# ZJU-FAST-Lab/uneven_planner

Hardware: AMD Instinct MI355X
Metric: MINCO traj-opts/sec (batch) (higher is better)
Workload: dtype f64

## Files before the change

uneven_planner_amd/csrc/solver_program.hpp:

```cpp
#pragma once
#include "terrain_dev.hpp"
#include "trajectory_dev.hpp"
#include "uph_common.hpp"

namespace uph {

#ifndef UPH_GRID_FROM_MEM
#define UPH_GRID_FROM_MEM 1
#endif
#ifndef UPH_PHASE_MASK
#define UPH_PHASE_MASK 15
#endif
#ifndef UPH_STATE_PROBE
#define UPH_STATE_PROBE(st) do { } while (0)
#endif
#ifndef UPH_SCALING_WB
#define UPH_SCALING_WB 8
#endif
#ifndef UPH_SC_XB
#define UPH_SC_XB 9
#endif
#ifndef UPH_SC_YB
#define UPH_SC_YB 14
#endif
#ifndef UPH_SC_WLO
#define UPH_SC_WLO 2
#endif
#ifndef UPH_SC_WHI
#define UPH_SC_WHI 3
#endif

#ifndef UPH_ASIDE_PREP
#define UPH_ASIDE_PREP 1
#endif
template <class WG, class F>
UPH_HD void asideKnotSolve(WG& wg, int lenW, int lenX, int n, F f) {
    (void)lenW; (void)lenX;
    wg.pfor(n, f);
}

template <class WG, class SR = double>
struct Solver {
    WG& wg;
    const GridDev& grid;
    const OptParams& P;
    const BatchDev& bd;
    const TrajDesc& td;
    int Nxy, Nyaw, n, S, K, mem, CH, CHP, recd;
    int CHS;
    int* rtag;
    double *x, *xp, *g, *gp, *d, *cxy, *cyaw, *Gxy, *Gyaw, *gamxy, *gamyaw, *bt, *rec, *wtab, *ttab, *pf, *hd;
    double* ab;
    int* abn;
    static constexpr int AB_DOUBLES = 4;
    double* up;
    static constexpr int UP_DOUBLES = 6;
    UPH_HD void tally(int k, bool yes) {
#if defined(__HIP_DEVICE_COMPILE__)
        if (yes && wg.wave == 0) abn[k] = abn[k] + 1;
#else
        if (yes) abn[k]++;
#endif
    }
    double *dual, *res, *scl, *hist;
    int hrow, hnp;
    const double *Wr_xy, *Wr_yaw;
    double rho, scale_fx, Txy, Tyaw, last_jerk, last_gd;
    long long hist_reads;
    long long cyc[16];
    long long t_last_eval_end;
    long long* sub_t = nullptr;
    int evals, bidx, trace_n;
    float inv_k1;
    double ec_irho, ec_step, ec_invK, ec_iTyaw, ec_omega, ec_omega_h;

    static constexpr int REC_FIELDS = 12;
    static UPH_HD size_t ldsDoubles(int Nxy, int Nyaw, int n, int CH, int mem, int K) {
        size_t recd = (size_t)REC_FIELDS * (CH + 1) + (CH + 1) / 2;
        const size_t nvec = 2 * (Nxy + 5) + (Nyaw + 5);
        const size_t knd = (size_t)knotBufDoubles(Nxy + 1, 4) + knotBufDoubles(Nyaw + 1, 2), adj = (size_t)knotBufDoubles(Nxy, 4) + knotBufDoubles(Nyaw, 2) + nvec;
        recd = recd < knd ? knd : recd;
        recd = recd < adj ? adj : recd;
        recd = recd < (size_t)mem ? (size_t)mem : recd;
        const size_t td_ = (size_t)Nxy + K + 2;
        return (size_t)5 * n + (nvec < td_ ? td_ : nvec) + 2 * (12 * Nxy + 6 * Nyaw) + recd + (size_t)6 * (K + 1) + THOMAS_DOUBLES + MAX_PAST + 8 + 18 + AB_DOUBLES + UP_DOUBLES;
    }

    UPH_HD Solver(WG& w, const GridDev& gr, const OptParams& p, const BatchDev& b, int bi, double* lds)
        : wg(w), grid(gr), P(p), bd(b), td(b.desc[bi]) {
        bidx = bi;
        Nxy = td.Nxy; Nyaw = td.Nyaw; n = td.n; S = td.S; K = P.int_K; mem = P.mem_size;
        inv_k1 = 1.0f / (float)(K + 1);
        CH = wg.size(); CHP = CH + 1; recd = REC_FIELDS * CHP + (CH + 1) / 2;
        CHS = CH;
#if !defined(UPH_ALIGNED_CHUNKS) || UPH_ALIGNED_CHUNKS
        {
            const int ppc = CH / (K + 1);
            if (ppc >= 1 && (Nxy + ppc - 1) / ppc == (S + CH - 1) / CH) CHS = ppc * (K + 1);
        }
#endif
        double* q = lds;
        x = q; q += n; g = q; q += n; d = q; q += n;
        xp = q; q += n; gp = q; q += n;
        const int nvec = 2 * (Nxy + 5) + (Nyaw + 5);
        bt = q;
        gamxy = q; gamyaw = q + 2 * (Nxy + 5);
        q += nvec < Nxy + K + 2 ? Nxy + K + 2 : nvec;
        cxy = q; q += 12 * Nxy; cyaw = q; q += 6 * Nyaw;
        Gxy = q; q += 12 * Nxy; Gyaw = q; q += 6 * Nyaw;
        wtab = q; q += 6 * (K + 1);
        rec = q;
        {
            size_t rd = (size_t)recd;
            const size_t knd = (size_t)knotBufDoubles(Nxy + 1, 4) + knotBufDoubles(Nyaw + 1, 2), adj = (size_t)knotBufDoubles(Nxy, 4) + knotBufDoubles(Nyaw, 2) + nvec;
            rd = rd < knd ? knd : rd; rd = rd < adj ? adj : rd; rd = rd < (size_t)mem ? (size_t)mem : rd;
            q += rd;
        }
        rtag = (int*)(rec + (size_t)REC_FIELDS * CHP);
        ttab = q; q += THOMAS_DOUBLES;
        pf = q; q += MAX_PAST + 8;
        hd = q; q += 18;
        ab = q; q += AB_DOUBLES;
        abn = (int*)(ab + 1);
        up = q; q += UP_DOUBLES;
        dual = bd.dual + 7 * td.off_s; res = bd.res + 7 * td.off_s; scl = bd.scl + 7 * td.off_s;
        hist = bd.hist + td.off_hist; hrow = histRowDoubles(n); hnp = 64 * histNQ(n);
        Wr_xy = bd.ops[td.op_xy].Wr; Wr_yaw = bd.ops[td.op_yaw].Wr;
        rho = 0; scale_fx = 1.0; Txy = Tyaw = 0; last_jerk = 0; hist_reads = 0; evals = 0; trace_n = 0;
        for (int q = 0; q < 16; q++) cyc[q] = 0;
        t_last_eval_end = 0;
        wg.pfor(18 + THOMAS_DOUBLES, [&](int t) {
            if (t == 0) { ab[0] = 0.0; abn[0] = abn[1] = abn[2] = abn[3] = 0; }
            if (t < 18) hd[t] = t < 6 ? td.init_xy[t] : (t < 12 ? td.end_xy[t - 6] : (t < 15 ? td.init_yaw[t - 12] : td.end_yaw[t - 15]));
            else ttab[t - 18] = bd.thomas[t - 18];
        });
    }

    UPH_HD void tracePush(double v) {
        if (bd.trace != nullptr && trace_n < bd.trace_cap) {
            const int at = trace_n;
            wg.one([&]() { bd.trace[(size_t)bidx * bd.trace_cap + at] = v; });
        }
        trace_n++;
    }

    static UPH_HD int divSmall(int a, int b, float inv) {
        int q = (int)((float)a * inv);
        const int r = a - q * b;
        if (r < 0) q--;
        else if (r >= b) q++;
        return q;
    }
    static UPH_HD int knotCol(int j, int N) { return j == 0 ? 0 : (j == N ? N + 2 : j + 2); }
    UPH_HD double knotPos(const double* xin, int j, int dd) const {
        if (dd < 2) return j == 0 ? hd[dd] : (j == Nxy ? hd[6 + dd] : xin[1 + 2 * (j - 1) + dd]);
        return j == 0 ? hd[12] : (j == Nyaw ? hd[15] : xin[1 + 2 * (Nxy - 1) + (j - 1)]);
    }

    UPH_HD double dot(const double* a, const double* b, int m) {
// ... 996 lines not shown
            step = io->step; fx = io->fx; k = io->k; end = io->end; bound = io->bound; budget = io->budget;
            wg.pfor(n, [&](int i) { xp[i] = x[i]; gp[i] = g[i]; });
            dginit = dot(g, d, n);
        } else {
            fx = eval<false>(x, g);
            wg.pfor(n + 1, [&](int i) { if (i < n) { d[i] = -g[i]; xp[i] = x[i]; gp[i] = g[i]; } else pf[0] = fx; });
            const double gnorm0 = absmax(g, n), xnorm0 = absmax(x, n);
            if (gnorm0 / dmax(1.0, xnorm0) < P.g_epsilon) {
                ret = LBFGS_CONVERGENCE;
                run = false;
            } else {
                const double dd0 = dot(d, d, n);
                step = 1.0 / sqrt(dd0);
                dginit = -dd0;
                k = 1; end = 0; bound = 0;
            }
        }
        double gnorm_inf, xnorm_inf;
        if (run) {
            while (true) {
                if constexpr (RESUME) {
                    if (budget == 0) { ret = LBFGS_RUNNING_HOOK; break; }
                    budget--;
                }
                ls = lineSearch(fx, step, P.min_step, P.max_step, dginit);
                if (ls < 0) {
                    wg.pfor(n, [&](int i) { x[i] = xp[i]; g[i] = gp[i]; });
                    ret = ls;
                    break;
                }
                tracePush(fx);
                if (k > 1000) { ret = LBFGS_CANCELED; break; }
                double* hr = hist + (size_t)end * hrow;
                double* sc = hr + 2;
                double* yc = hr + 2 + hnp;
                const double pf_old = (0 < P.past && P.past <= k) ? wg.bcast(pf[k % P.past]) : 0.0;
                UPH_MARK("lbfgs.bookkeeping");
                double r5[5], mx2[2];
                wg.template sumMax<5, 2>(n, r5, mx2, [&](int i, double* acc, double* mx) {
                    const double xv = x[i], gv = g[i], xo = xp[i], go = gp[i];
                    const double sv = xv - xo, yv = gv - go;
                    mx[0] = dmax(mx[0], fabs(gv)); mx[1] = dmax(mx[1], fabs(xv));
                    sc[i] = sv; yc[i] = yv;
                    acc[0] += yv * sv; acc[1] += yv * yv; acc[2] += sv * sv; acc[3] += go * go; acc[4] += gv * gv;
                    xp[i] = xv; gp[i] = gv;
                    d[i] = -gv;
                });
                gnorm_inf = mx2[0];
                xnorm_inf = mx2[1];
                if (gnorm_inf / dmax(1.0, xnorm_inf) < P.g_epsilon) { ret = LBFGS_CONVERGENCE; break; }
                if (0 < P.past) {
                    if (P.past <= k) {
                        const double rate = fabs(pf_old - fx) / dmax(1.0, fabs(fx));
                        if (rate < P.delta) { ret = LBFGS_STOP; break; }
                    }
                }
                if (P.inner_max_iter != 0 && P.inner_max_iter <= k) { ret = LBFGSERR_MAXIMUMITERATION; break; }
                ys = r5[0]; yy = r5[1];
                const double cau = r5[2] * sqrt(r5[3]) * P.cautious_factor;
                {
                    const int kk = k, e0 = end;
                    const double fv = fx, ysv = ys;
                    wg.pfor(1, [&](int) {
                        if (0 < P.past) pf[kk % P.past] = fv;
                        double* h0 = hist + (size_t)e0 * hrow;
                        h0[0] = ysv; h0[1] = 1.0 / ysv;
                    });
                }
// ... 151 lines not shown
            st.f = io.fx; st.last_lbfgs_ret = ret; st.lbfgs_iters = io.k;
        });
        storeTrajectory(st);
    }

    UPH_HD void microbench(TrajState& st, int reps) {
        const double* gx0 = bd.x + td.off_x;
        rho = wg.bcast(st.rho); scale_fx = wg.bcast(st.scale_fx);
        wg.pfor(n, [&](int t) { x[t] = gx0[t]; d[t] = 0.5; xp[t] = gx0[t]; gp[t] = 0.25; });
        long long a[9];
        long long sub[8] = {0, 0, 0, 0, 0, 0, 0, 0};
        sub_t = sub;
        double acc = 0.0, js[3], part[3], c1, c2;
        const int cnt = S < CH ? S : CH;
        a[0] = wg.clock();
        for (int r = 0; r < reps; r++) generate<false>(x, 0.0);
        a[1] = wg.clock();
        for (int r = 0; r < reps; r++) { expand(x, 1.0, js); acc += js[0]; }
        a[2] = wg.clock();
        for (int r = 0; r < reps; r++) evalConsts(evalStep());
        a[3] = wg.clock();
        for (int r = 0; r < reps; r++) { wg.template sum<3>(cnt, part, [&](int t, double* ac) { sampleEval<false>(t, t, ac); }); acc += part[0]; }
        a[4] = wg.clock();
        for (int r = 0; r < reps; r++) scatterChunk(0, cnt);
        a[5] = wg.clock();
        for (int r = 0; r < reps; r++) { adjoint(c1, c2); acc += c1 + c2; }
        a[6] = wg.clock();
        const int m = mem;
        for (int r = 0; r < reps; r++) {
            const int end = (r * 7) % m, bound = m;
            acc += absmax(g, n) + absmax(x, n);
            wg.sync();
            wg.pfor(1, [&](int) { pf[r % 3] = acc; });
            double* sc = hist + (size_t)end * hrow + 2;
            double* yc = sc + hnp;
            double r6[6] = {0, 0, 0, 0, 0, 0};
            wg.template sum<3>(n, r6, [&](int i, double* ac) {
                const double sv = x[i] - xp[i], yv = g[i] - gp[i];
                sc[i] = sv; yc[i] = yv;
                ac[0] += yv * sv; ac[1] += yv * yv; ac[2] += sv * sv;
                d[i] = -g[i];
            });
            acc += r6[0] + r6[3] + sqrt(dot(gp, gp, n));
            wg.sync();
            wg.pfor(1, [&](int) { hist[(size_t)end * hrow] = acc; });
            (void)bound;
        }
        a[7] = wg.clock();
        wg.pfor(1, [&](int) {
            for (int q = 0; q < 7; q++) st.cyc[q] = (a[q + 1] - a[q]) / reps;
            st.cyc[7] = a[7] - a[0];
            for (int q = 0; q < 8; q++) st.cyc[8 + q] = sub[q] / reps;
            st.f = acc;
        });
        sub_t = nullptr;
    }

    UPH_HD void evalOnly(TrajState& st, int repeat) {
        const double* gx0 = bd.x + td.off_x;
        rho = wg.bcast(st.rho); scale_fx = wg.bcast(st.scale_fx);
        wg.pfor(n, [&](int t) { x[t] = gx0[t]; });
        double f = 0.0;
        for (int r = 0; r < repeat; r++) f = eval<false>(x, g);
        refreshResiduals();
        wg.pfor(n, [&](int t) { bd.gout[td.off_x + t] = g[t]; });
        storeTrajectory(st);
        wg.pfor(1, [&](int) { st.f = f; });
    }
// ... 89 lines not shown
```

uneven_planner_amd/csrc/unevenhip.hip:

```cpp
#include <hip/hip_runtime.h>

#include <type_traits>

#include <algorithm>
#include <cmath>
#include <cstdio>
#include <cstdlib>
#include <cstring>
#include <map>
#include <numeric>
#include <string>
#include <thread>
#include <vector>

#include "../../include/uneven_hip.h"
#include "minco_op_host.hpp"
#include "resample_walk.hpp"
#include "solver_program.hpp"
#include "uph_ctx.hpp"
#include "wave_dev.hpp"

using namespace uph;

#ifndef UPH_THOMAS_KPL
// ... 181 lines not shown
#pragma unroll
            for (int w = 1; w < NW; w++) t += r[w * MAXM + m];
            outS[m] = uni(t);
        }
#pragma unroll
        for (int m = 0; m < MM; m++) {
            double t = r[MS + m];
#pragma unroll
            for (int w = 1; w < NW; w++) t = r[w * MAXM + MS + m] > t ? r[w * MAXM + MS + m] : t;
            outM[m] = uni(t);
        }
    }
    __device__ __forceinline__ double bcast(double v) const { return uni(v); }
    static __device__ __forceinline__ double divByStored(double x, double ys, double r) {
        const double q0 = x * r;
        return fma(fma(-q0, ys, x), r, q0);
    }
    template <int NQ, int PF>
    __device__ __forceinline__ void twoLoopT(double* d, const double* g, double* dg_out, double* al_lds, int n_, const double* hist_, int m_, int end_, int bound_, double scale_) {
        typedef double dbl2_t __attribute__((ext_vector_type(2)));
        typedef const __attribute__((address_space(1))) char* gbytes;
        constexpr int NP2 = NQ / 2;
        constexpr bool ODD = (NQ & 1) != 0;
        constexpr int NPAD = 64 * NQ, ROWB = (2 + 2 * NPAD) * 8;
        const gbytes hist = (gbytes)uniG(hist_);
        const int lane = flane();
        const int n = uni(n_), m = uni(m_), end = uni(end_), bound = uni(bound_);
        const double scale = uni(scale_);
        const unsigned l16 = 16u * (unsigned)lane, l8 = 8u * (unsigned)lane;
        auto eidx = [&](int q) { return q < 2 * NP2 ? 128 * (q >> 1) + 2 * lane + (q & 1) : 64 * (NQ - 1) + lane; };
        double dr[NQ], sr[PF][NQ], yr[PF][NQ], ysr[PF], rysr[PF];
#pragma unroll
        for (int q = 0; q < NQ; q++) { const int e = eidx(q); dr[q] = e < n ? d[e] : 0.0; }
        auto fetch = [&](int slot, int j) {
            const gbytes row = hist + (size_t)((unsigned)j * (unsigned)ROWB);
            const dbl2_t yr2 = *(const __attribute__((address_space(1))) dbl2_t*)row;
            ysr[slot] = yr2.x; rysr[slot] = yr2.y;
#pragma unroll
            for (int p = 0; p < NP2; p++) {
                const dbl2_t s2 = *(const __attribute__((address_space(1))) dbl2_t*)(row + 16 + 1024 * p + l16);
                const dbl2_t y2 = *(const __attribute__((address_space(1))) dbl2_t*)(row + 16 + NPAD * 8 + 1024 * p + l16);
                sr[slot][2 * p] = s2.x; sr[slot][2 * p + 1] = s2.y; yr[slot][2 * p] = y2.x; yr[slot][2 * p + 1] = y2.y;
            }
            if (ODD) {
                sr[slot][NQ - 1] = *(const __attribute__((address_space(1))) double*)(row + 16 + 512 * (NQ - 1) + l8);
                yr[slot][NQ - 1] = *(const __attribute__((address_space(1))) double*)(row + 16 + NPAD * 8 + 512 * (NQ - 1) + l8);
            }
        };
        auto rowDot = [&](const double* a, const double* b_) {
            if (NQ == 1) return a[0] * b_[0];
            if (NQ == 2) return fma(a[1], b_[1], a[0] * b_[0]);
            if (NQ == 3) return fma(a[2], b_[2], fma(a[1], b_[1], a[0] * b_[0]));
            if (NQ == 4) return fma(a[1], b_[1], a[0] * b_[0]) + fma(a[3 % NQ], b_[3 % NQ], a[2 % NQ] * b_[2 % NQ]);
            double e = a[0] * b_[0], o = a[1 % NQ] * b_[1 % NQ];
#pragma unroll
            for (int q = 2; q < NQ; q += 2) e = fma(a[q], b_[q], e);
#pragma unroll
            for (int q = 3; q < NQ; q += 2) o = fma(a[q], b_[q], o);
            return e + o;
        };
        auto step1 = [&](int u, int i) {
            const double al = divByStored(waveSum(rowDot(sr[u], dr)), ysr[u], rysr[u]);
            al_lds[i] = al;
#pragma unroll
            for (int q = 0; q < NQ; q++) dr[q] = fma(-al, yr[u][q], dr[q]);
        };
        auto step2 = [&](int u, int i) {
            const double alpha = al_lds[bound - 1 - i];
            const double beta = divByStored(waveSum(rowDot(yr[u], dr)), ysr[u], rysr[u]);
            const double a = alpha - beta;
#pragma unroll
            for (int q = 0; q < NQ; q++) dr[q] = fma(a, sr[u][q], dr[q]);
        };
        auto pin = [&]() {
#pragma unroll
            for (int q = 0; q < NQ; q++) asm volatile("" : "+v"(dr[q]) : : "memory");
        };
#ifdef UPH_TL_PROF
        const long long tp0 = __builtin_readcyclecounter();
#endif
        int jf = end;
// ... 181 lines not shown
            __builtin_amdgcn_s_setprio(3);
            constexpr int PF = UPH_TWOLOOP_PF;
            const int nq = uni((n + 63) >> 6);
            if (nq == 1) twoLoopT<1, PF>(d, g, dg_out, al_lds, n, hist, m, end, bound, scale);
            else if (nq == 2) twoLoopT<2, PF>(d, g, dg_out, al_lds, n, hist, m, end, bound, scale);
            else if (nq == 3) twoLoopT<3, PF>(d, g, dg_out, al_lds, n, hist, m, end, bound, scale);
            else if (nq == 4) twoLoopT<4, PF>(d, g, dg_out, al_lds, n, hist, m, end, bound, scale);
            else if (nq == 5) twoLoopT<5, 2>(d, g, dg_out, al_lds, n, hist, m, end, bound, scale);
            else if (nq == 6) twoLoopT<6, 2>(d, g, dg_out, al_lds, n, hist, m, end, bound, scale);
            else if (nq == 7) twoLoopT<7, 2>(d, g, dg_out, al_lds, n, hist, m, end, bound, scale);
            else twoLoopT<8, 2>(d, g, dg_out, al_lds, n, hist, m, end, bound, scale);
            __builtin_amdgcn_s_setprio(0);
        }
        bar(1);
    }
    template <class F>
    __device__ __forceinline__ double maxv(int n, F f) {
        double a = 0.0;
        for (int i = ftid(); i < n; i += NT) { const double v = f(i); a = v > a ? v : a; }
        a = waveMax(a);
        double* r = red + par * (NW * MAXM);
        par ^= 1;
        if (lane == 0) r[wave * MAXM] = a;
        bar(0);
        double t = r[0];
#pragma unroll
        for (int w = 1; w < NW; w++) t = r[w * MAXM] > t ? r[w * MAXM] : t;
        return uni(t);
    }
};

template <int NT, class F>
__device__ __forceinline__ void asideKnotSolve(DevWG<NT>& wg, int lenW, int lenX, int n, F f) { wg.aside(lenW, lenX, n, f); }

template <int NT, int WPS, int MODE, bool F32S = false>
__global__ __launch_bounds__(NT, WPS) void uph_solver_kernel(GridDev grid, OptParams P, BatchDev bd, int repeat) {
    extern __shared__ double lds[];
    const int w = blockIdx.x;
    if (w >= bd.B) return;
    const int b = bd.order ? bd.order[w] : w;
    DevWG<NT> wg(lds);
    typedef typename std::conditional<F32S, f32r, double>::type SR;
    Solver<DevWG<NT>, SR> sol(wg, grid, P, bd, b, lds + DevWG<NT>::SCRATCH);
    TrajState& st = bd.state[b];
    if (MODE == 0) sol.evalOnly(st, repeat);
    else if (MODE == 1) sol.prepare(st);
    else if (MODE == 2) sol.optimize(st, repeat);
    else if (MODE == 7) sol.resumeHook(st, repeat >> 1, repeat & 1);
    else if (MODE == 8) { if (repeat & 1) sol.template penaltyOnly<true>(st, repeat >> 1); else sol.template penaltyOnly<false>(st, repeat >> 1); }
    else if (MODE == 3) sol.report(st);
    else if (MODE == 5) sol.microbench(st, repeat);
    else sol.scalingOnly(st);
}

__global__ void uph_fill_kernel(double* __restrict__ p, size_t n, double v) {
    for (size_t i = (size_t)blockIdx.x * blockDim.x + threadIdx.x; i < n; i += (size_t)gridDim.x * blockDim.x) p[i] = v;
}

__global__ void uph_terrain_kernel(GridDev grid, const double* __restrict__ pos, int n, double* __restrict__ values, double* __restrict__ grads) {
    const int i = blockIdx.x * blockDim.x + threadIdx.x;
    if (i >= n) return;
    const double yaw = pos[3 * i + 2];
    double v[7], g[7][3];
    terrainAllWithGrad(grid, pos[3 * i], pos[3 * i + 1], yaw, cos(yaw), sin(yaw), v, g);
    for (int k = 0; k < 7; k++) {
        values[7 * i + k] = v[k];
// ... 253 lines not shown
        else if (mode == 2) UPH_LAUNCH(NTL, WPS, 2);                                                                                 \
        else if (mode == 3) UPH_LAUNCH(NTL, WPS, 3);                                                                                 \
        else if (mode == 5) UPH_LAUNCH(NTL, WPS, 5);                                                                                 \
        else UPH_LAUNCH(NTL, WPS, 4);                                                                                                \
    } while (0)
#define UPH_LAUNCH32(NTL, WPS, MODE)                                                                                                   \
    do {                                                                                                                             \
        const size_t ldsmax = 160 * 1024;    \
        HIPCHK(hipFuncSetAttribute((const void*)uph_solver_kernel<NTL, WPS, MODE, true>, hipFuncAttributeMaxDynamicSharedMemorySize, (int)ldsmax)); \
        HIPCHK(hipEventRecord(evb, c->stream));                                                                                   \
        BatchDev bm = bd;                                                                                                            \
        bm.B = c->n_main;                                                                                                            \
        if (c->n_main < c->B) {                                                                                                      \
            BatchDev bb = bd;                                                                                                        \
            bb.B = c->B - c->n_main;                                                                                                 \
            bb.order = bd.order + c->n_main;                                                                                         \
            HIPCHK(hipStreamWaitEvent(c->stream2, evb, 0));                                                                       \
            hipLaunchKernelGGL((uph_solver_kernel<NTL, WPS, MODE, true>), dim3(bb.B), dim3(NTL), c->lds_big, c->stream2, grid, c->P, bb, repeat); \
            HIPCHK(hipEventRecord(c->ev2, c->stream2));                                                                              \
        }                                                                                                                            \
        hipLaunchKernelGGL((uph_solver_kernel<NTL, WPS, MODE, true>), dim3(c->n_main), dim3(NTL), c->lds_bytes, c->stream, grid, c->P, bm, repeat); \
        if (c->n_main < c->B) HIPCHK(hipStreamWaitEvent(c->stream, c->ev2, 0));                                                      \
    } while (0)
    if (c->sample_f32 && (mode == 0 || mode == 2) && (c->lanes == 128 || c->lanes == 256 || c->lanes == 512)) {
        if (c->lanes == 128) { if (mode == 0) UPH_LAUNCH32(128, 2, 0); else UPH_LAUNCH32(128, 2, 2); }
        else if (c->lanes == 512) { if (mode == 0) UPH_LAUNCH32(512, 1, 0); else UPH_LAUNCH32(512, 1, 2); }
        else if (mode == 0) UPH_LAUNCH32(256, 1, 0);
        else if (c->wps == 2 && c->lds_bytes <= 80 * 1024) UPH_LAUNCH32(256, 2, 2);
        else UPH_LAUNCH32(256, 1, 2);
    }
    else if (mode == 7) {
        if (c->lanes == 128) UPH_LAUNCH(128, 2, 7);
        else if (c->lanes == 256) UPH_LAUNCH(256, 1, 7);
        else { setError("the L-BFGS resume hook is built for 128 and 256 lanes"); return UPH_ERR_INVALID; }
    }
    else if (mode == 8) {
        if (c->lanes == 128) UPH_LAUNCH(128, 2, 8);
        else if (c->lanes == 256) UPH_LAUNCH(256, 1, 8);
        else if (c->lanes == 512) UPH_LAUNCH(512, 1, 8);
        else UPH_LAUNCH(64, 1, 8);
    }
    else if (c->lanes == 64 && c->wps_forced == 2) UPH_LAUNCH_MODE(64, 2);
    else if (c->lanes == 64) UPH_LAUNCH_MODE(64, 1);
    else if (c->lanes == 128 && mode == 1) UPH_LAUNCH(128, 1, 1);
    else if (c->lanes == 128) UPH_LAUNCH_MODE(128, UPH_WPS128);
    else if (c->lanes == 512) UPH_LAUNCH_MODE(512, 1);
    else if (c->wps == 2 && mode == 2 && c->lds_bytes <= 80 * 1024) UPH_LAUNCH(256, 2, 2);
    else if (c->wps == 2 && mode == 5 && c->lds_bytes <= 80 * 1024) UPH_LAUNCH(256, 2, 5);
    else UPH_LAUNCH_MODE(256, 1);
#undef UPH_LAUNCH_MODE
#undef UPH_LAUNCH32
#undef UPH_LAUNCH
    HIPCHK(hipGetLastError());
    if (mode == 0 || mode == 2 || mode == 4 || mode == 7) c->traj_resident = true;
    HIPCHK(hipEventRecord(eve, c->stream));
    if (async) return UPH_OK;
    HIPCHK(hipStreamSynchronize(c->stream));
    float ms = 0.f;
    HIPCHK(hipEventElapsedTime(&ms, evb, eve));
    c->last_ms = ms;
    return UPH_OK;
}

static int uploadPackedX(uph_ctx* c, const double* x_packed) {
    if (c->frames.empty()) { HIPCHK(hipMemcpy(c->d_x.p, x_packed, 8 * c->sum_n, hipMemcpyHostToDevice)); return UPH_OK; }
    std::vector<double> xl(x_packed, x_packed + c->sum_n);
    for (int b = 0; b < c->B; b++) {
// ... 188 lines not shown
    c->frames.clear();
    c->framed_valid = false;
    c->frames_grid = tg;
    if (std::max(std::max(std::fabs(tg.minb[0]), std::fabs(tg.maxb[0])), std::max(std::fabs(tg.minb[1]), std::fabs(tg.maxb[1]))) > FRAME_EXTENT) {
        c->frames.resize(B);
        for (int b = 0; b < B; b++) {
            const ProblemHead& q = *pp[b];
            TrajFrame& f = c->frames[b];
            const int nn[2] = {tg.nx, tg.ny};
            for (int d = 0; d < 2; d++) {
                long long ci = std::llround((0.5 * (q.lo[d] + q.hi[d]) - tg.origin[d]) * tg.xy_inv);
                ci = ci < 0 ? 0 : (ci > nn[d] ? nn[d] : ci);
                f.ioff[d] = (int)ci;
                f.shift[d] = tg.origin[d] + (double)ci * tg.xy_res;
                f.fo[d] = 0.0;
                f.lo[d] = tg.lo[d] - f.shift[d];
                f.hi[d] = tg.hi[d] - f.shift[d];
            }
        }
    }
    for (int b = 0; b < B; b++) {
        const ProblemHead& pr = *pp[b];
        const int Nxy = pr.n_inner_xy + 1, Nyaw = pr.n_inner_yaw + 1;
        TrajDesc& t = c->desc[b];
        std::memset(&t, 0, sizeof(t));
        t.Nxy = Nxy; t.Nyaw = Nyaw; t.n = 2 * pr.n_inner_xy + pr.n_inner_yaw + 1; t.S = Nxy * K1;
        t.op_xy = ensureOp(c, Nxy);
        t.op_yaw = ensureOp(c, Nyaw);
        if (t.op_xy < 0 || t.op_yaw < 0) return UPH_ERR_HIP;
        t.off_x = on; t.off_s = os; t.off_cxy = ocx; t.off_cyaw = ocy; t.off_hist = oh;
        for (int k = 0; k < 6; k++) { t.init_xy[k] = pr.init_xy[k]; t.end_xy[k] = pr.end_xy[k]; }
        for (int k = 0; k < 3; k++) { t.init_yaw[k] = pr.init_yaw[k]; t.end_yaw[k] = pr.end_yaw[k]; }
        if (!c->frames.empty()) for (int d = 0; d < 2; d++) { t.init_xy[d] -= c->frames[b].shift[d]; t.end_xy[d] -= c->frames[b].shift[d]; }
        on += t.n; os += t.S; ocx += 12 * Nxy; ocy += 6 * Nyaw; oh += (int64_t)mem * histRowDoubles(t.n);
        c->fp_bytes[b] = (Solver<DevWG<64>>::ldsDoubles(Nxy, Nyaw, t.n, c->lanes, mem, c->P.int_K) + 2 * (c->lanes / 64) * DevWG<64>::MAXM) * sizeof(double);
        lds_d = std::max(lds_d, Solver<DevWG<64>>::ldsDoubles(Nxy, Nyaw, t.n, c->lanes, mem, c->P.int_K));
    }
    c->sum_n = on; c->sum_S = os; c->sum_cxy = ocx; c->sum_cyaw = ocy; c->sum_hist = oh;
    c->lds_bytes = (lds_d + 2 * (c->lanes / 64) * DevWG<64>::MAXM) * sizeof(double);
    if (c->lds_bytes > 160 * 1024) { setError("uph_batch_upload: trajectory does not fit the 160 KiB LDS"); return UPH_ERR_LIMIT; }
    if (c->ops_dirty) {
        if (c->d_ops.ensure(sizeof(MincoOp) * c->ops_host.size())) return UPH_ERR_HIP;
        HIPCHK(hipMemcpy(c->d_ops.p, c->ops_host.data(), sizeof(MincoOp) * c->ops_host.size(), hipMemcpyHostToDevice));
        c->ops_dirty = false;
    }
    if (c->d_desc.ensure(sizeof(TrajDesc) * B) || c->d_state.ensure(sizeof(TrajState) * B) || c->d_x.ensure(8 * on) || c->d_x0.ensure(8 * on) || c->d_gout.ensure(8 * on) ||
        c->d_dual.ensure(8 * 7 * os) || c->d_res.ensure(8 * 7 * os) || c->d_scl.ensure(8 * 7 * os) || c->d_cxy.ensure(8 * ocx) || c->d_cyaw.ensure(8 * ocy) ||
        c->d_hist.ensure(8 * oh) || c->d_report.ensure(8 * 7 * B) || c->d_order.ensure(4 * B) ||
        c->d_trace.ensure(8 * (size_t)std::max(1, c->trace_cap) * B))
        return UPH_ERR_HIP;
    {
        std::vector<double> cost(B);
        for (int b = 0; b < B; b++) cost[b] = predictedCostOf(pp[b]->n_inner_xy, pp[b]->n_inner_yaw, pp[b]->turn, pp[b]->kink);
        c->order.resize(B);
        std::iota(c->order.begin(), c->order.end(), 0);
        std::stable_sort(c->order.begin(), c->order.end(), [&](int a, int b2) { return cost[a] > cost[b2]; });
        if (c->xcd_group >= 16) {
            const GridDev gg = uphMapGrid(c->map);
            auto octant = [&](int b) {
                const ProblemHead& q = *pp[b];
                const double mx = 0.5 * (q.init_xy[0] + q.end_xy[0]), my = 0.5 * (q.init_xy[1] + q.end_xy[1]);
                const int ix = mx < 0.5 * (gg.minb[0] + gg.maxb[0]) ? 0 : 1;
                int iy = (int)((my - gg.minb[1]) / (gg.maxb[1] - gg.minb[1]) * 4.0);
                iy = iy < 0 ? 0 : (iy > 3 ? 3 : iy);
                return ix * 4 + iy;
            };
            const int G = c->xcd_group & ~7;
// ... 675 lines not shown
        c->last_abandon[0] += s.ls_rejected; c->last_abandon[1] += s.ls_guarded; c->last_abandon[2] += s.ls_abandoned;
        c->last_abandon[3] += s.chunks_skipped; c->last_abandon[4] += s.adjoints_skipped;
        c->last_iters += s.lbfgs_iters;
        c->last_hist_bytes += s.hist_reads * 8;
    }
}
int uph_batch_set_x(uph_ctx* c, const double* x_packed) {
    if (c && c->pending) { setError("an asynchronous solve is in flight on this context: call uph_batch_wait first"); return UPH_ERR_INVALID; }
    if (c && c->n_rejected) { setError("packed-array hooks need a batch without unsupported problems (uph_result.ret_code == UPH_RET_UNSUPPORTED)"); return UPH_ERR_INVALID; }
    if (!c || c->B <= 0 || !x_packed) { setError("uph_batch_set_x: bad arguments"); return UPH_ERR_INVALID; }
    HIPCHK(hipSetDevice(c->device));
    return uploadPackedX(c, x_packed);
}
int uph_batch_alm_passes(uph_ctx* c, int32_t max_passes) {
    if (!c || c->B <= 0 || max_passes < 0) { setError("uph_batch_alm_passes: bad arguments"); return UPH_ERR_INVALID; }
    int r = launchSolver(c, 2, max_passes);
    if (r != UPH_OK) return r;
    r = refreshStates(c);
    if (r != UPH_OK) return r;
    collectSolveStats(c);
    return UPH_OK;
}
int uph_batch_set_lbfgs_state(uph_ctx* c, const double* g, const double* d, const double* pf, const double* lm_s, const double* lm_y, const double* lm_ys, const double* scal5) {
    if (c && c->pending) { setError("an asynchronous solve is in flight on this context: call uph_batch_wait first"); return UPH_ERR_INVALID; }
    if (c && c->n_rejected) { setError("packed-array hooks need a batch without unsupported problems (uph_result.ret_code == UPH_RET_UNSUPPORTED)"); return UPH_ERR_INVALID; }
    if (!c || c->B <= 0 || !g || !d || !pf || !lm_s || !lm_y || !lm_ys || !scal5) { setError("uph_batch_set_lbfgs_state: bad arguments"); return UPH_ERR_INVALID; }
    HIPCHK(hipSetDevice(c->device));
    const int mem = c->P.mem_size;
    if (c->d_rsd.ensure(8 * c->sum_n) || c->d_rs.ensure(8 * 24 * (size_t)c->B)) return UPH_ERR_HIP;
    std::vector<double> hist((size_t)c->sum_hist, 0.0), rs((size_t)24 * c->B, 0.0);
    int64_t off = 0;
    for (int b = 0; b < c->B; b++) {
        const TrajDesc& t = c->desc[b];
        const int rowd = histRowDoubles(t.n), np = 64 * histNQ(t.n);
        for (int j = 0; j < mem; j++) {
            double* row = hist.data() + t.off_hist + (size_t)j * rowd;
            const double ys = lm_ys[(size_t)b * mem + j];
            row[0] = ys; row[1] = 1.0 / ys;
            std::memcpy(row + 2, lm_s + off + (size_t)j * t.n, 8 * t.n);
            std::memcpy(row + 2 + np, lm_y + off + (size_t)j * t.n, 8 * t.n);
        }
        off += (int64_t)mem * t.n;
        for (int q = 0; q < 5; q++) rs[(size_t)24 * b + q] = scal5[5 * b + q];
        for (int q = 0; q < UPH_MAX_PAST; q++) rs[(size_t)24 * b + 8 + q] = pf[(size_t)b * UPH_MAX_PAST + q];
    }
    HIPCHK(hipMemcpy(c->d_hist.p, hist.data(), 8 * c->sum_hist, hipMemcpyHostToDevice));
    HIPCHK(hipMemcpy(c->d_rs.p, rs.data(), 8 * rs.size(), hipMemcpyHostToDevice));
    HIPCHK(hipMemcpy(c->d_gout.p, g, 8 * c->sum_n, hipMemcpyHostToDevice));
    HIPCHK(hipMemcpy(c->d_rsd.p, d, 8 * c->sum_n, hipMemcpyHostToDevice));
    return UPH_OK;
}
int uph_batch_lbfgs_resume(uph_ctx* c, int32_t budget, int32_t finish_pass) {
    if (!c || c->B <= 0 || !c->d_rs.p) { setError("uph_batch_lbfgs_resume: no state set"); return UPH_ERR_INVALID; }
    const int bud = budget < 0 ? (1 << 28) : budget;
    int r = launchSolver(c, 7, 2 * bud + (finish_pass ? 1 : 0));
    if (r != UPH_OK) return r;
    r = refreshStates(c);
    if (r != UPH_OK) return r;
    collectSolveStats(c);
    return UPH_OK;
}
int uph_batch_get_lbfgs_state(uph_ctx* c, double* g, double* d, double* pf, double* lm_s, double* lm_y, double* lm_ys, double* scal8) {
    if (c && c->pending) { setError("an asynchronous solve is in flight on this context: call uph_batch_wait first"); return UPH_ERR_INVALID; }
    if (!c || c->B <= 0 || !c->d_rs.p) { setError("uph_batch_get_lbfgs_state: no state set"); return UPH_ERR_INVALID; }
    HIPCHK(hipSetDevice(c->device));
    const int mem = c->P.mem_size;
    std::vector<double> hist((size_t)c->sum_hist), rs((size_t)24 * c->B);
    HIPCHK(hipMemcpy(hist.data(), c->d_hist.p, 8 * c->sum_hist, hipMemcpyDeviceToHost));
    HIPCHK(hipMemcpy(rs.data(), c->d_rs.p, 8 * rs.size(), hipMemcpyDeviceToHost));
    if (g) HIPCHK(hipMemcpy(g, c->d_gout.p, 8 * c->sum_n, hipMemcpyDeviceToHost));
    if (d) HIPCHK(hipMemcpy(d, c->d_rsd.p, 8 * c->sum_n, hipMemcpyDeviceToHost));
    int64_t off = 0;
    for (int b = 0; b < c->B; b++) {
        const TrajDesc& t = c->desc[b];
        const int rowd = histRowDoubles(t.n), np = 64 * histNQ(t.n);
        for (int j = 0; j < mem; j++) {
            const double* row = hist.data() + t.off_hist + (size_t)j * rowd;
            if (lm_ys) lm_ys[(size_t)b * mem + j] = row[0];
            if (lm_s) std::memcpy(lm_s + off + (size_t)j * t.n, row + 2, 8 * t.n);
            if (lm_y) std::memcpy(lm_y + off + (size_t)j * t.n, row + 2 + np, 8 * t.n);
        }
        off += (int64_t)mem * t.n;
        if (scal8) for (int q = 0; q < 8; q++) scal8[8 * b + q] = rs[(size_t)24 * b + q];
        if (pf) for (int q = 0; q < UPH_MAX_PAST; q++) pf[(size_t)b * UPH_MAX_PAST + q] = rs[(size_t)24 * b + 8 + q];
    }
    return UPH_OK;
}

int uph_terrain_query(uph_map* m, const double* pos, int32_t n, double* values7, double* grads21) {
    if (!m || !pos || n <= 0 || !values7 || !grads21) { setError("uph_terrain_query: bad arguments"); return UPH_ERR_INVALID; }
    HIPCHK(hipSetDevice(uphMapDevice(m)));
    UphPtr tp, tv, tg;
    tp.p = uphMapScratch(m, 0, 8 * 3 * (size_t)n); tv.p = uphMapScratch(m, 1, 8 * 7 * (size_t)n); tg.p = uphMapScratch(m, 2, 8 * 21 * (size_t)n);
    if (!tp.p || !tv.p || !tg.p) return UPH_ERR_HIP;
    HIPCHK(hipMemcpy(tp.p, pos, 8 * 3 * (size_t)n, hipMemcpyHostToDevice));
    hipLaunchKernelGGL(uph_terrain_kernel, dim3((n + 255) / 256), dim3(256), 0, 0, uphMapGrid(m), tp.as<double>(), n, tv.as<double>(), tg.as<double>());
    HIPCHK(hipGetLastError());
    HIPCHK(hipDeviceSynchronize());
    HIPCHK(hipMemcpy(values7, tv.p, 8 * 7 * (size_t)n, hipMemcpyDeviceToHost));
    HIPCHK(hipMemcpy(grads21, tg.p, 8 * 21 * (size_t)n, hipMemcpyDeviceToHost));
    return UPH_OK;
}

}
#endif
```

uneven_planner_amd/csrc/uph_common.hpp:

```cpp
#pragma once
#include <math.h>
#include <stdint.h>

#if defined(__HIPCC__)
#define UPH_HD __host__ __device__ __forceinline__
#define UPH_NOINLINE __host__ __device__ __attribute__((noinline))
#else
#define UPH_HD inline
#define UPH_NOINLINE __attribute__((noinline))
#endif

#if defined(__HIP_DEVICE_COMPILE__)
#define UPH_AS_GLOBAL(p) ((const __attribute__((address_space(1))) double*)(p))
#else
#define UPH_AS_GLOBAL(p) (p)
#endif

#if defined(UPH_ISA_MARKS) && defined(__HIP_DEVICE_COMPILE__)
#define UPH_MARK(name) asm volatile("; UPHMARK " name)
#else
#define UPH_MARK(name) do { } while (0)
#endif

namespace uph {
// ... 136 lines not shown
};

#if defined(__HIP_DEVICE_COMPILE__)
UPH_HD void pinv(double& v) { asm volatile("" : "+v"(v)); }
UPH_HD void pinv(float& v) { asm volatile("" : "+v"(v)); }
UPH_HD void pinv(int& v) { asm volatile("" : "+v"(v)); }
#else
UPH_HD void pinv(double&) {}
UPH_HD void pinv(float&) {}
UPH_HD void pinv(int&) {}
#endif
#ifndef UPH_DIET
#define UPH_DIET 0
#endif

UPH_HD double dmax(double a, double b) { return a > b ? a : b; }
UPH_HD double dmin(double a, double b) { return a < b ? a : b; }

UPH_HD double expC2(double tau) { return tau > 0.0 ? ((0.5 * tau + 1.0) * tau + 1.0) : 1.0 / ((0.5 * tau - 1.0) * tau + 1.0); }
UPH_HD double divR(double x, double y, double r) {
    const double q0 = x * r;
    return fma(fma(-q0, y, x), r, q0);
}
UPH_HD void mv2(const double* M, double v0, double v1, double& o0, double& o1) {
    o0 = fma(M[1], v1, M[0] * v0);
    o1 = fma(M[3], v1, M[2] * v0);
}
UPH_HD void submv2(double r0, double r1, const double* M, double p0, double p1, double& o0, double& o1) {
    o0 = fma(-M[1], p1, fma(-M[0], p0, r0));
    o1 = fma(-M[3], p1, fma(-M[2], p0, r1));
}
UPH_HD int histNQ(int n) { return (n + 63) >> 6; }
UPH_HD int histRowDoubles(int n) { return 2 + 128 * histNQ(n); }
constexpr int THOMAS_J = 26;
constexpr int THOMAS_STRIDE = 8;
constexpr int THOMAS_DOUBLES = (THOMAS_J + 1) * THOMAS_STRIDE;
constexpr int THOMAS_KPL = 4;
UPH_HD int knotOff(int q, int ks) { return ks * q + (q >> 2); }
UPH_HD int knotOffJ(int j, int ks) { return ks * j + ((j + 3) >> 2); }
UPH_HD int knotBufDoubles(int nknots, int ks) { return ks * nknots + (nknots >> 2) + 2; }
template <bool ADJ>
UPH_HD void thomasFactors(const double* tab, int j, double* P, double* M1, double* Q, double* M2) {
    const double* e = tab + (j < THOMAS_J ? j : THOMAS_J) * THOMAS_STRIDE;
    const double* en = tab + (j + 1 < THOMAS_J ? j + 1 : THOMAS_J) * THOMAS_STRIDE;
    const double D00 = e[4], D01 = e[5], D10 = e[6], D11 = e[7];
    if (!ADJ) {
        P[0] = 1.0; P[1] = 0.0; P[2] = 0.0; P[3] = 1.0;
        M1[0] = e[0]; M1[1] = e[1]; M1[2] = e[2]; M1[3] = e[3];
        Q[0] = D00; Q[1] = D01; Q[2] = D10; Q[3] = D11;
        M2[0] = fma(8.0, D00, -7.0 * D01); M2[1] = D01 - D00; M2[2] = fma(8.0, D10, -7.0 * D11); M2[3] = D11 - D10;
    } else {
        P[0] = D00; P[1] = D10; P[2] = D01; P[3] = D11;
        const double z = j == 1 ? 0.0 : 1.0;
        M1[0] = z * fma(8.0, D00, -D10); M1[1] = z * fma(-7.0, D00, D10); M1[2] = z * fma(8.0, D01, -D11); M1[3] = z * fma(-7.0, D01, D11);
        Q[0] = 1.0; Q[1] = 0.0; Q[2] = 0.0; Q[3] = 1.0;
        M2[0] = en[0]; M2[1] = en[2]; M2[2] = en[1]; M2[3] = en[3];
    }
}
#if defined(__HIP_DEVICE_COMPILE__)
static __device__ __constant__ const double UPH_SINCOS_TAB[16] = {
#else
static const double UPH_SINCOS_TAB[16] = {
#endif
    0x1.45f306dc9c883p-1,
    0x1.921fb54442d18p+0, 0x1.1a62633145c07p-54, -0x1.f1976b7ed8fbcp-110,
    -1.66666666666666324348e-01, 8.33333333332248946124e-03, -1.98412698298579493134e-04,
// ... 99 lines not shown
```

Before: 54090.

## Pack L-BFGS history rows compactly instead of padding to 64-element groups

```diff
diff --git a/uneven_planner_amd/csrc/solver_program.hpp b/uneven_planner_amd/csrc/solver_program.hpp
--- a/uneven_planner_amd/csrc/solver_program.hpp
+++ b/uneven_planner_amd/csrc/solver_program.hpp
@@ -37,6 +37,12 @@
 UPH_HD void asideKnotSolve(WG& wg, int lenW, int lenX, int n, F f) {
     (void)lenW; (void)lenX;
     wg.pfor(n, f);
+}
+
+template <class WG>
+UPH_HD HistRowLayout histRowLayout(WG& wg, int n) {
+    (void)wg;
+    return histLayoutPadded(n);
 }
 
 template <class WG, class SR = double>
@@ -63,7 +69,7 @@
 #endif
     }
     double *dual, *res, *scl, *hist;
-    int hrow, hnp;
+    int hrow, hoff_s, hoff_y;
     const double *Wr_xy, *Wr_yaw;
     double rho, scale_fx, Txy, Tyaw, last_jerk, last_gd;
     long long hist_reads;
@@ -124,7 +130,8 @@
         abn = (int*)(ab + 1);
         up = q; q += UP_DOUBLES;
         dual = bd.dual + 7 * td.off_s; res = bd.res + 7 * td.off_s; scl = bd.scl + 7 * td.off_s;
-        hist = bd.hist + td.off_hist; hrow = histRowDoubles(n); hnp = 64 * histNQ(n);
+        hist = bd.hist + td.off_hist;
+        { const HistRowLayout hl = histRowLayout(wg, n); hrow = hl.stride; hoff_s = hl.off_s; hoff_y = hl.off_y; }
         Wr_xy = bd.ops[td.op_xy].Wr; Wr_yaw = bd.ops[td.op_yaw].Wr;
         rho = 0; scale_fx = 1.0; Txy = Tyaw = 0; last_jerk = 0; hist_reads = 0; evals = 0; trace_n = 0;
         for (int q = 0; q < 16; q++) cyc[q] = 0;
@@ -1187,8 +1194,8 @@
                 tracePush(fx);
                 if (k > 1000) { ret = LBFGS_CANCELED; break; }
                 double* hr = hist + (size_t)end * hrow;
-                double* sc = hr + 2;
-                double* yc = hr + 2 + hnp;
+                double* sc = hr + hoff_s;
+                double* yc = hr + hoff_y;
                 const double pf_old = (0 < P.past && P.past <= k) ? wg.bcast(pf[k % P.past]) : 0.0;
                 UPH_MARK("lbfgs.bookkeeping");
                 double r5[5], mx2[2];
@@ -1406,8 +1413,8 @@
             acc += absmax(g, n) + absmax(x, n);
             wg.sync();
             wg.pfor(1, [&](int) { pf[r % 3] = acc; });
-            double* sc = hist + (size_t)end * hrow + 2;
-            double* yc = sc + hnp;
+            double* sc = hist + (size_t)end * hrow + hoff_s;
+            double* yc = hist + (size_t)end * hrow + hoff_y;
             double r6[6] = {0, 0, 0, 0, 0, 0};
             wg.template sum<3>(n, r6, [&](int i, double* ac) {
                 const double sv = x[i] - xp[i], yv = g[i] - gp[i];
diff --git a/uneven_planner_amd/csrc/unevenhip.hip b/uneven_planner_amd/csrc/unevenhip.hip
--- a/uneven_planner_amd/csrc/unevenhip.hip
+++ b/uneven_planner_amd/csrc/unevenhip.hip
@@ -237,6 +237,33 @@
         double dr[NQ], sr[PF][NQ], yr[PF][NQ], ysr[PF], rysr[PF];
 #pragma unroll
         for (int q = 0; q < NQ; q++) { const int e = eidx(q); dr[q] = e < n ? d[e] : 0.0; }
+#if UPH_HIST_COMPACT
+        constexpr int NFULL = ODD ? NP2 : NP2 - 1;
+        const HistRowLayout hl = histLayoutCompact(n);
+        const unsigned rowb = 8u * (unsigned)hl.stride, ybyte = 8u * (unsigned)hl.off_y;
+        int lastS = histLaneByte(n, 0, lane, NP2 - (ODD ? 0 : 1)), lastY = histLaneByte(n, 1, lane, NP2 - (ODD ? 0 : 1));
+        pinv(lastS); pinv(lastY);
+        auto fetch = [&](int slot, int j) {
+            const gbytes row = hist + (size_t)((unsigned)j * rowb);
+            const gbytes rowy = row + ybyte;
+            const dbl2_t yr2 = *(const __attribute__((address_space(1))) dbl2_t*)row;
+            ysr[slot] = yr2.x; rysr[slot] = yr2.y;
+#pragma unroll
+            for (int p = 0; p < NFULL; p++) {
+                const dbl2_t s2 = *(const __attribute__((address_space(1))) dbl2_t*)(row + 32 + 1024 * p + l16);
+                const dbl2_t y2 = *(const __attribute__((address_space(1))) dbl2_t*)(rowy + 1024 * p + l16);
+                sr[slot][2 * p] = s2.x; sr[slot][2 * p + 1] = s2.y; yr[slot][2 * p] = y2.x; yr[slot][2 * p + 1] = y2.y;
+            }
+            if (ODD) {
+                sr[slot][NQ - 1] = *(const __attribute__((address_space(1))) double*)(row + (unsigned)lastS);
+                yr[slot][NQ - 1] = *(const __attribute__((address_space(1))) double*)(row + (unsigned)lastY);
+            } else {
+                const dbl2_t s2 = *(const __attribute__((address_space(1))) dbl2_t*)(row + (unsigned)lastS);
+                const dbl2_t y2 = *(const __attribute__((address_space(1))) dbl2_t*)(row + (unsigned)lastY);
+                sr[slot][NQ - 2] = s2.x; sr[slot][NQ - 1] = s2.y; yr[slot][NQ - 2] = y2.x; yr[slot][NQ - 1] = y2.y;
+            }
+        };
+#else
         auto fetch = [&](int slot, int j) {
             const gbytes row = hist + (size_t)((unsigned)j * (unsigned)ROWB);
             const dbl2_t yr2 = *(const __attribute__((address_space(1))) dbl2_t*)row;
@@ -252,6 +279,7 @@
                 yr[slot][NQ - 1] = *(const __attribute__((address_space(1))) double*)(row + 16 + NPAD * 8 + 512 * (NQ - 1) + l8);
             }
         };
+#endif
         auto rowDot = [&](const double* a, const double* b_) {
             if (NQ == 1) return a[0] * b_[0];
             if (NQ == 2) return fma(a[1], b_[1], a[0] * b_[0]);
@@ -499,6 +527,8 @@
 
 template <int NT, class F>
 __device__ __forceinline__ void asideKnotSolve(DevWG<NT>& wg, int lenW, int lenX, int n, F f) { wg.aside(lenW, lenX, n, f); }
+template <int NT>
+UPH_HD HistRowLayout histRowLayout(DevWG<NT>& wg, int n) { (void)wg; return histLayoutDevice(n); }
 
 template <int NT, int WPS, int MODE, bool F32S = false>
 __global__ __launch_bounds__(NT, WPS) void uph_solver_kernel(GridDev grid, OptParams P, BatchDev bd, int repeat) {
@@ -818,7 +848,8 @@
     else if (mode == 7) {
         if (c->lanes == 128) UPH_LAUNCH(128, 2, 7);
         else if (c->lanes == 256) UPH_LAUNCH(256, 1, 7);
-        else { setError("the L-BFGS resume hook is built for 128 and 256 lanes"); return UPH_ERR_INVALID; }
+        else if (c->lanes == 512) UPH_LAUNCH(512, 1, 7);
+        else UPH_LAUNCH(64, 1, 7);
     }
     else if (mode == 8) {
         if (c->lanes == 128) UPH_LAUNCH(128, 2, 8);
@@ -1073,7 +1104,7 @@
         for (int k = 0; k < 6; k++) { t.init_xy[k] = pr.init_xy[k]; t.end_xy[k] = pr.end_xy[k]; }
         for (int k = 0; k < 3; k++) { t.init_yaw[k] = pr.init_yaw[k]; t.end_yaw[k] = pr.end_yaw[k]; }
         if (!c->frames.empty()) for (int d = 0; d < 2; d++) { t.init_xy[d] -= c->frames[b].shift[d]; t.end_xy[d] -= c->frames[b].shift[d]; }
-        on += t.n; os += t.S; ocx += 12 * Nxy; ocy += 6 * Nyaw; oh += (int64_t)mem * histRowDoubles(t.n);
+        on += t.n; os += t.S; ocx += 12 * Nxy; ocy += 6 * Nyaw; oh += (int64_t)mem * histLayoutDevice(t.n).stride;
         c->fp_bytes[b] = (Solver<DevWG<64>>::ldsDoubles(Nxy, Nyaw, t.n, c->lanes, mem, c->P.int_K) + 2 * (c->lanes / 64) * DevWG<64>::MAXM) * sizeof(double);
         lds_d = std::max(lds_d, Solver<DevWG<64>>::ldsDoubles(Nxy, Nyaw, t.n, c->lanes, mem, c->P.int_K));
     }
@@ -1815,13 +1846,13 @@
     int64_t off = 0;
     for (int b = 0; b < c->B; b++) {
         const TrajDesc& t = c->desc[b];
-        const int rowd = histRowDoubles(t.n), np = 64 * histNQ(t.n);
+        const HistRowLayout hl = histLayoutDevice(t.n);
         for (int j = 0; j < mem; j++) {
-            double* row = hist.data() + t.off_hist + (size_t)j * rowd;
+            double* row = hist.data() + t.off_hist + (size_t)j * hl.stride;
             const double ys = lm_ys[(size_t)b * mem + j];
             row[0] = ys; row[1] = 1.0 / ys;
-            std::memcpy(row + 2, lm_s + off + (size_t)j * t.n, 8 * t.n);
-            std::memcpy(row + 2 + np, lm_y + off + (size_t)j * t.n, 8 * t.n);
+            std::memcpy(row + hl.off_s, lm_s + off + (size_t)j * t.n, 8 * t.n);
+            std::memcpy(row + hl.off_y, lm_y + off + (size_t)j * t.n, 8 * t.n);
         }
         off += (int64_t)mem * t.n;
         for (int q = 0; q < 5; q++) rs[(size_t)24 * b + q] = scal5[5 * b + q];
@@ -1856,12 +1887,12 @@
     int64_t off = 0;
     for (int b = 0; b < c->B; b++) {
         const TrajDesc& t = c->desc[b];
-        const int rowd = histRowDoubles(t.n), np = 64 * histNQ(t.n);
+        const HistRowLayout hl = histLayoutDevice(t.n);
         for (int j = 0; j < mem; j++) {
-            const double* row = hist.data() + t.off_hist + (size_t)j * rowd;
+            const double* row = hist.data() + t.off_hist + (size_t)j * hl.stride;
             if (lm_ys) lm_ys[(size_t)b * mem + j] = row[0];
-            if (lm_s) std::memcpy(lm_s + off + (size_t)j * t.n, row + 2, 8 * t.n);
-            if (lm_y) std::memcpy(lm_y + off + (size_t)j * t.n, row + 2 + np, 8 * t.n);
+            if (lm_s) std::memcpy(lm_s + off + (size_t)j * t.n, row + hl.off_s, 8 * t.n);
+            if (lm_y) std::memcpy(lm_y + off + (size_t)j * t.n, row + hl.off_y, 8 * t.n);
         }
         off += (int64_t)mem * t.n;
         if (scal8) for (int q = 0; q < 8; q++) scal8[8 * b + q] = rs[(size_t)24 * b + q];
diff --git a/uneven_planner_amd/csrc/uph_common.hpp b/uneven_planner_amd/csrc/uph_common.hpp
--- a/uneven_planner_amd/csrc/uph_common.hpp
+++ b/uneven_planner_amd/csrc/uph_common.hpp
@@ -192,6 +192,23 @@
 }
 UPH_HD int histNQ(int n) { return (n + 63) >> 6; }
 UPH_HD int histRowDoubles(int n) { return 2 + 128 * histNQ(n); }
+#ifndef UPH_HIST_COMPACT
+#define UPH_HIST_COMPACT 1
+#endif
+struct HistRowLayout { int stride, off_s, off_y; };
+constexpr int HIST_ZERO_BYTE = 16;
+UPH_HD HistRowLayout histLayoutPadded(int n) { return HistRowLayout{histRowDoubles(n), 2, 2 + 64 * histNQ(n)}; }
+UPH_HD HistRowLayout histLayoutCompact(int n) {
+    const int np = (n + 1) & ~1;
+    return HistRowLayout{(4 + 2 * np + 15) & ~15, 4, 4 + np};
+}
+UPH_HD HistRowLayout histLayoutDevice(int n) { return UPH_HIST_COMPACT ? histLayoutCompact(n) : histLayoutPadded(n); }
+UPH_HD int histLaneByte(int n, int region, int lane, int grp) {
+    const HistRowLayout L = histLayoutCompact(n);
+    const int nq = histNQ(n);
+    const int e = grp < nq / 2 ? 128 * grp + 2 * lane : 64 * (nq - 1) + lane;
+    return e < n ? 8 * ((region ? L.off_y : L.off_s) + e) : HIST_ZERO_BYTE;
+}
 constexpr int THOMAS_J = 26;
 constexpr int THOMAS_STRIDE = 8;
 constexpr int THOMAS_DOUBLES = (THOMAS_J + 1) * THOMAS_STRIDE;
```

New measurement: 54540, median of 6. Within noise of the previous version (+0.8%).
